# timoblak/sq-recovery

Hardware: NVIDIA B200
Metric: fused SQ implicit-loss fwd+bwd throughput (higher is better)
Workload: dtype f32

## Files before the change

sq_recovery_b200/counting.py:

```python
from __future__ import annotations

import ctypes
import os

import torch

from . import _lib
from .functional import nearest_offsets

LIB_COUNT = os.path.join(_lib.HERE, "libsqloss_count.so")
_h = None

XU_PER_EVENT = {"plane_steps": 11, "spot_backward_blocks": 5, "dealout_rounds": 13, "refine_rounds": 11,
                "column_groups": 16, "items": 6}
NAMES = ("plane_steps", "spot_backward_blocks", "dealout_rounds", "refine_rounds", "items", "column_groups",
         "queued_points", "refined_points")


def lib():
    global _h
    if _h is None:
        if not os.path.exists(LIB_COUNT):
            raise RuntimeError(f"{LIB_COUNT} not found: python -m sq_recovery_b200.build")
        h = ctypes.CDLL(LIB_COUNT)
        for name, (res, args) in _lib._PROTOS.items():
            fn = getattr(h, name)
            fn.restype, fn.argtypes = res, args
        h.sq_debug_counters.restype = ctypes.c_int
        h.sq_debug_counters.argtypes = [ctypes.c_void_p, ctypes.c_int]
        _h = h
    return _h


def implicit_counts(images: torch.Tensor, pred: torch.Tensor, n: int, tau: float, sharpness: float, want_grad: bool = True):
    h = lib()
    dev = pred.device
    B = pred.shape[0]
    p = pred.detach().float().contiguous()
    img = images.detach().float().contiguous()
    row_off, col_off = nearest_offsets(img.shape[2], img.shape[3], n, dev)
    nb = h.sq_scratch_bytes(B, n)
    scratch = torch.zeros(nb, dtype=torch.uint8, device=dev)
    loss = torch.empty((), dtype=torch.float64, device=dev)
    grad = torch.empty_like(p) if want_grad else None
    P = lambda t: ctypes.c_void_p(t.data_ptr()) if t is not None else None
    cnt = (ctypes.c_ulonglong * 8)()
    torch.cuda.synchronize()
    _lib.check(h.sq_debug_counters(cnt, 1), "sq_debug_counters")
    rc = h.sq_implicit_loss(P(p), _lib.SQ_F32, B, n, 1.0 / (n - 1), 1e-4, P(img), img.shape[2] * img.shape[3], P(row_off),
                            P(col_off), tau, sharpness, P(loss), None, P(grad), None, P(scratch), nb,
                            torch.cuda.current_stream(dev).cuda_stream)
    _lib.check(rc, "sq_implicit_loss (counting build)")
    torch.cuda.synchronize()
    _lib.check(h.sq_debug_counters(cnt, 1), "sq_debug_counters")
    c = dict(zip(NAMES, (int(v) for v in cnt)))
    grid_points = B * n ** 3
    xu = sum(XU_PER_EVENT[k] * c[k] for k in XU_PER_EVENT)
    return {"counters": c, "grid_points": grid_points, "point_evaluations": 32 * c["plane_steps"],
            "walked_fraction": 32 * c["plane_steps"] / grid_points, "xu_warp_inst_model": xu,
            "loss": loss.item()}
```

sq_recovery_b200/csrc/sq_core.cuh:

```cuda
#pragma once
#include <math.h>
#include <stdint.h>
#include <string.h>

#if defined(__CUDACC__)
#define SQ_HD __host__ __device__ __forceinline__
#else
#define SQ_HD inline
#endif

#if !defined(__CUDACC__)
struct float2 { float x, y; };
#endif

#ifndef SQ_COUNT_HOOK
#define SQ_COUNT_HOOK(i, n) do { } while (0)
#endif

namespace sq {

constexpr float kLog2e = 1.4426950408889634f;
constexpr double kLn2 = 0.6931471805599453;
constexpr float kAbsFix = 1e-2f;
#ifndef SQ_KACTIVE
// ... 37 lines not shown
#else
    return log2f(fabsf(x));
#endif
}
SQ_HD float ex2_neg_abs(float x) {
#if defined(__CUDA_ARCH__)
    float y; asm("{\n .reg .f32 t;\n abs.f32 t, %1;\n neg.f32 t, t;\n ex2.approx.ftz.f32 %0, t;\n}" : "=f"(y) : "f"(x)); return y;
#else
    return exp2f(-fabsf(x));
#endif
}

struct Grid {
    int n;
    double step;
    double z0;
    float inv_n;
    float stepf, z0f;
};
SQ_HD Grid make_grid(int n, double step, double z0) {
    Grid g; g.n = n; g.step = step; g.z0 = z0; g.inv_n = 1.0f / (float)n; g.stepf = (float)step; g.z0f = (float)z0; return g;
}
SQ_HD double grid_coord(const Grid& g, int i) { return i == 0 ? g.z0 : (double)i * g.step; }
SQ_HD float grid_coord_f32(const Grid& g, int i) { return i == 0 ? g.z0f : (float)i * g.stepf; }

SQ_HD float d2f(double v) {
#if defined(__CUDA_ARCH__)
    float y; asm("cvt.rn.f32.f64 %0, %1;" : "=f"(y) : "d"(v)); return y;
#else
    return (float)v;
#endif
}
SQ_HD double f2d(float v) {
#if defined(__CUDA_ARCH__)
    double y; asm("cvt.f64.f32 %0, %1;" : "=d"(y) : "f"(v)); return y;
#else
    return (double)v;
#endif
}

struct Sample {
    double Ms[9];
    double t[3];
    float mf[6];
    float of[3];
    float dh[3], dl[3];
    float idh[3];
    float cf0;
    float pxy, pz;
    float e21, e1;
    float wd[3];
    float qw, qa, qia, qB1;
    int zpack;
    double pxy64, pz64, e21_64, e1_64;
};
struct SampleFull : Sample {
    double M[9];
    double a[3], e[2], q[4];
    double ia[3];
    double hp[8], hrn;
    int heads, pad2_;
    float mask[8];
};

SQ_HD void split2(double v, float& hi, float& lo) { hi = d2f(v); lo = d2f(v - f2d(hi)); }

SQ_HD void heads_forward(const double* raw, double* p, double* hp, double& hrn) {
    for (int i = 0; i < 8; ++i) { hp[i] = (double)(float)(1.0 / (1.0 + exp(-raw[i]))); p[i] = hp[i]; }
    const double n2 = raw[8] * raw[8] + raw[9] * raw[9] + raw[10] * raw[10] + raw[11] * raw[11];
    hrn = 1.0 / sqrt(n2);
    for (int i = 8; i < 12; ++i) p[i] = (double)(float)(raw[i] * hrn);
}
SQ_HD void heads_backward(const double* hp, double hrn, const double* q, double* gr) {
    for (int i = 0; i < 8; ++i) gr[i] *= hp[i] * (1.0 - hp[i]);
    const double dot = q[0] * gr[8] + q[1] * gr[9] + q[2] * gr[10] + q[3] * gr[11];
    for (int i = 0; i < 4; ++i) gr[8 + i] = (gr[8 + i] - q[i] * dot) * hrn;
}

SQ_HD double clamped_param(const double* p, bool clamp, int i, float* mask = nullptr) {
    const double lo = i < 3 ? 0.05 : (i < 5 ? 0.1 : 0.0);
    double x = p[i];
    float m = 1.0f;
    if (clamp) {
        if (x < lo) { x = lo; m = 0.0f; }
        if (x > 1.0) { x = 1.0; m = 0.0f; }
    }
    if (mask) *mask = m;
    return x;
}
SQ_HD void prep_part(const double* p, bool clamp, const Grid& g, SampleFull& S, int part) {
    if (part < 3) {
        const int i = part;
        const double x = -p[8], y = -p[9], z = -p[10], w = p[11];
        const double tx = 2.0 * x, ty = 2.0 * y, tz = 2.0 * z;
        const double twx = tx * w, twy = ty * w, twz = tz * w;
        const double txx = tx * x, txy = ty * x, txz = tz * x;
        const double tyy = ty * y, tyz = tz * y, tzz = tz * z;
        double m0, m1, m2;
        if (i == 0)      { m0 = 1.0 - (tyy + tzz); m1 = txy - twz;         m2 = txz + twy; }
        else if (i == 1) { m0 = txy + twz;         m1 = 1.0 - (txx + tzz); m2 = tyz - twx; }
        else             { m0 = txz - twy;         m1 = tyz + twx;         m2 = 1.0 - (txx + tyy); }
        S.M[3 * i] = m0; S.M[3 * i + 1] = m1; S.M[3 * i + 2] = m2;
        const double a = clamped_param(p, clamp, i);
        const double t0 = clamped_param(p, clamp, 5), t1 = clamped_param(p, clamp, 6), t2 = clamped_param(p, clamp, 7);
        const double ia = 1.0 / a;
        S.ia[i] = ia;
        const double s0 = m0 * ia, s1 = m1 * ia, s2 = m2 * ia;
        S.Ms[3 * i] = s0; S.Ms[3 * i + 1] = s1; S.Ms[3 * i + 2] = s2;
        split2(s2 * g.step, S.dh[i], S.dl[i]);
        S.idh[i] = 1.0f / S.dh[i];
        S.mf[2 * i] = (float)s0; S.mf[2 * i + 1] = (float)s1;
        S.of[i] = (float)-(s0 * t0 + s1 * t1 + s2 * t2);
    } else {
        const double e1 = clamped_param(p, clamp, 3), e2 = clamped_param(p, clamp, 4);
        const double w1 = e2 > 0.0 ? (e2 < 1.0 ? exp2(e2 - 1.0) : 1.0) : 0.0;
        const double b1 = e1 > 0.0 ? (e1 < 1.0 ? exp2(1.0 - e1) : 1.0) : 1e30;
        S.qw = (float)w1; S.qB1 = (float)b1;
        S.pxy64 = 2.0 / e2; S.pz64 = 2.0 / e1; S.e21_64 = e2 / e1; S.e1_64 = e1;
        S.pxy = (float)S.pxy64; S.pz = (float)S.pz64; S.e21 = (float)S.e21_64; S.e1 = (float)e1;
        S.cf0 = (float)(g.z0 / g.step);
    }
}
SQ_HD int zero_planes(const SampleFull& S, const Grid& g) {
    int pack = 0;
    for (int i = 0; i < 3; ++i) {
        if (S.M[3 * i] != 0.0 || S.M[3 * i + 1] != 0.0 || S.M[3 * i + 2] == 0.0) continue;
        const double m = S.M[3 * i + 2], target = m * S.t[2];
        const int c0 = (int)(S.t[2] / g.step + 0.5);
        for (int c = c0 - 1; c <= c0 + 1; ++c) {
            if (c < 1 || c >= g.n || c > 1023) continue;
            if (m * grid_coord(g, c) == target) pack |= c << (10 * i);
        }
    }
    return pack;
}
SQ_HD float round13(float v) {
    int b;
#if defined(__CUDA_ARCH__)
    b = __float_as_int(v);
#else
    memcpy(&b, &v, 4);
#endif
    b = (b + 0x400) & ~0x7ff;
#if defined(__CUDA_ARCH__)
    return __int_as_float(b);
#else
    float r; memcpy(&r, &b, 4); return r;
#endif
}
SQ_HD void resplit_zero_rows(SampleFull& S, const Grid& g) {
    for (int i = 0; i < 3; ++i) {
        if (!((S.zpack >> (10 * i)) & 1023)) continue;
        const double d = S.Ms[3 * i + 2] * g.step;
        S.dh[i] = round13(d2f(d));
        S.dl[i] = round13(d2f(d - f2d(S.dh[i])));
        S.idh[i] = 1.0f / S.dh[i];
    }
}

SQ_HD void prep_finish(const double* p, bool clamp, const Grid& g, SampleFull& S) {
    for (int i = 0; i < 8; ++i) {
        float m;
        const double v = clamped_param(p, clamp, i, &m);
        S.mask[i] = m;
        if (i < 3) S.a[i] = v; else if (i < 5) S.e[i - 3] = v; else S.t[i - 5] = v;
    }
    for (int i = 0; i < 4; ++i) S.q[i] = p[8 + i];
    S.zpack = zero_planes(S, g);
    if (S.zpack) resplit_zero_rows(S, g);
    S.heads = 0; S.pad2_ = 0; S.hrn = 1.0;
    for (int i = 0; i < 8; ++i) S.hp[i] = 0.0;
    double al = 0.0;
    for (int i = 0; i < 3; ++i) {
// ... 326 lines not shown
    {
        const float r = sqrtf(bound * bound * 1.004f * S.qB1) + sqrtf(he2);
        const float beta = fmaf(S.wd[0], bc[0], fmaf(S.wd[1], bc[1], S.wd[2] * bc[2]));
        const float gamma = fmaf(S.qw, fmaf(bc[0], bc[0], bc[1] * bc[1]), fmaf(bc[2], bc[2], -r * r));
        const float disc = fmaf(beta, beta, -S.qa * gamma);
        const float sq = sqrtf(fmaxf(disc, 0.0f));
        lo = fmaxf(lo, (-beta - sq) * S.qia);
        hi = fminf(hi, disc > 0.0f ? (sq - beta) * S.qia : -1e30f);
    }
    const float nf = (float)g.n;
    lo = fminf(fmaxf(lo - 1.0f, 0.0f), nf);
    hi = fmaxf(fminf(hi + 1.0f, nf - 1.0f), -1.0f);
    const int c_lo = (int)ceilf(lo), c_hi = (int)floorf(hi);
    if (range_lo) *range_lo = c_lo;
    return c_hi >= c_lo ? c_hi - c_lo + 1 : 0;
}

SQ_HD int footprint_walk(const Sample& S, const Grid& g, float bound, float die, float cx, float cy, float hx, float hy) {
    int c_lo = 0;
    const int planes = footprint_planes(S, g, bound, cx, cy, hx, hy, &c_lo);
    if (planes <= 0 || !(die > 0.f)) return planes;
    const float a = fmaf(S.dh[0], S.dh[0], fmaf(S.dh[1], S.dh[1], S.dh[2] * S.dh[2])), ia = 1.0f / a, nf = (float)(g.n - 1);
    float stop = 1e30f;
    for (int k = 0; k < 4; ++k) {
        const float gx = (cx + ((k & 1) ? hx : -hx)) * g.stepf, gy = (cy + ((k & 2) ? hy : -hy)) * g.stepf;
        float b[3];
        for (int i = 0; i < 3; ++i) b[i] = fmaf(S.mf[2 * i], gx, fmaf(S.mf[2 * i + 1], gy, S.of[i]));
        const float beta = fmaf(S.dh[0], b[0], fmaf(S.dh[1], b[1], S.dh[2] * b[2]));
        const float gamma = fmaf(b[0], b[0], fmaf(b[1], b[1], fmaf(b[2], b[2], -0.97f)));
        const float disc = fmaf(beta, beta, -a * gamma);
        float s = (float)c_lo;
        if (disc > 0.f) {
            const float sq = sqrtf(disc);
            const float far_ = fmaxf((-beta - sq) * ia, 0.f), near_ = fminf((sq - beta) * ia, nf);
            if (near_ - far_ >= die) s = fmaxf(near_ - die - 1.0f, (float)c_lo);
        }
        stop = fminf(stop, s);
    }
    const int cut = (int)(stop - (float)c_lo);
    return cut > 0 ? (planes - cut > 1 ? planes - cut : 1) : planes;
}

SQ_HD void xfast_group_footprint(int n, int group, float& cx, float& cy, float& hx, float& hy) {
    const int first = group * 32;
    int last = first + 31;
    if (last > n * n - 1) last = n * n - 1;
    const int ib0 = first / n, ia0 = first - ib0 * n, ib1 = last / n, ia1 = last - ib1 * n;
    if (ib1 == ib0) { cx = 0.5f * (float)(ia0 + ia1); hx = 0.5f * (float)(ia1 - ia0); cy = (float)ib0; hy = 0.f; }
    else { cx = 0.5f * (float)(n - 1); hx = cx; cy = 0.5f * (float)(ib0 + ib1); hy = 0.5f * (float)(ib1 - ib0); }
}

#if defined(__CUDA_ARCH__)
#define SQ_ANY(p) __any_sync(0xffffffffu, (p))
#define SQ_BALLOT(p) __ballot_sync(0xffffffffu, (p))
#define SQ_WARP_MAX(v) __reduce_max_sync(0xffffffffu, (v))
#define SQ_WARP_MIN(v) __reduce_min_sync(0xffffffffu, (v))
#else
#define SQ_ANY(p) (p)
#define SQ_BALLOT(p) ((p) ? 1u : 0u)
#define SQ_WARP_MAX(v) (v)
#define SQ_WARP_MIN(v) (v)
#endif
SQ_HD unsigned lanes_below() {
#if defined(__CUDA_ARCH__)
    unsigned m; asm("mov.u32 %0, %%lanemask_lt;" : "=r"(m)); return m;
#else
    return 0u;
#endif
}
SQ_HD int popcount(unsigned m) {
#if defined(__CUDA_ARCH__)
    return __popc(m);
#else
    return __builtin_popcount(m);
#endif
}

SQ_HD void warp_range(int n, int& c_lo, int& c_hi) {
    const bool empty = c_hi < c_lo;
    c_hi = SQ_WARP_MAX(empty ? -1 : c_hi);
    c_lo = SQ_WARP_MIN(empty ? n : c_lo);
    if (c_hi < c_lo) { c_lo = 0; c_hi = -1; }
}

SQ_HD bool column_zero_possible(const Sample& S, const float* bh) {
    bool m = false;
    for (int i = 0; i < 3; ++i) {
        const float cs = -bh[i] * S.idh[i];
        const float r = cs - rintf(cs);
        m = m || !(fabsf(r) > 1e-4f) || !(fabsf(cs - S.cf0) > 1e-4f);
    }
    return m;
}

struct ImplicitParams { float kl; float tl; float bound; float kact; };
SQ_HD float implicit_active_bits(float kl, int n, int batch) {
    const float band = (260.0f * kLog2e / kl) * ((float)n / 64.0f);
    float bits = kActive + (band > 1.0f ? log2f(band) : 0.0f);
    const float point = log2f(kl * 1e9f / ((float)n * (float)n * (float)(batch > 0 ? batch : 1)));
    if (point > bits) bits = point;
    return bits < kImplicitCullBits ? bits : kImplicitCullBits;
}

#ifndef SQ_KDEEP
#define SQ_KDEEP 32.0f
#endif
constexpr float kDeep = SQ_KDEEP;

struct ColGrad {
    float gs0[3], gs1[3], gz0[3], gz1[3], ge0[2], ge1[2];
};

struct BwdQueue {
    float* cf;
    float* pre;
    float* x;
    float* d;
    int cap;
    int lane;
    unsigned where;
};
constexpr int kNoLink = 255;
constexpr unsigned kTagMask = 0x1fffu;
constexpr int kPoolMaxPlanes = 1024;

SQ_HD unsigned f32_bits(float v) {
#if defined(__CUDA_ARCH__)
    return __float_as_uint(v);
#else
    unsigned u; memcpy(&u, &v, 4); return u;
#endif
}
SQ_HD float bits_f32(unsigned u) {
#if defined(__CUDA_ARCH__)
    return __uint_as_float(u);
#else
    float v; memcpy(&v, &u, 4); return v;
#endif
}
SQ_HD float entry_cf(const Sample& S, float tagged) {
    const float cf = bits_f32(f32_bits(tagged) & ~kTagMask);
    return cf < 1.0f ? S.cf0 : cf;
}
SQ_HD int entry_lane(float tagged) { return (int)(f32_bits(tagged) & 31u); }
SQ_HD int entry_link(float tagged) { return (int)((f32_bits(tagged) >> 5) & 255u); }

struct ColState {
    float csl, cssum, tsum, psh, seen, T;
    BwdQueue q;
    int nr, top, head;
    bool spilled;
};

#if !defined(SQ_NO_BWD_COMPACT) && !defined(SQ_BWD_COMPACT)
// ... 106 lines not shown
                    if (active) {
#if defined(__CUDA_ARCH__)
                        const unsigned lane_ = st.q.where & 31u;
                        const int rank = popcount((shell ? ms : mp) & ((1u << lane_) - 1u));
                        const int at = shell ? st.nr + rank : st.top - rank;
                        const unsigned tag = lane_ | ((unsigned)(shell ? st.head : kNoLink) << 5);
                        const unsigned addr = (st.q.where & ~31u) + 4u * (unsigned)at;
                        asm volatile("st.shared.b32 [%0], %1;\n\tst.shared.f32 [%0 + %4], %2;\n\tst.shared.f32 [%0 + %5], %3;"
                                     :: "r"(addr), "r"((f32_bits(p.cf) & ~kTagMask) | tag), "f"(st.psh),
                                        "f"(shell ? p.x : p.eo * p.o * p.o), "n"(4 * kBwdPool), "n"(8 * kBwdPool) : "memory");
#else
                        const int rank = popcount((shell ? ms : mp) & lanes_below());
                        const int at = shell ? st.nr + rank : st.top - rank;
                        const unsigned tag = (unsigned)st.q.lane | ((unsigned)(shell ? st.head : kNoLink) << 5);
                        st.q.cf[at] = bits_f32((f32_bits(p.cf) & ~kTagMask) | tag);
                        st.q.pre[at] = st.psh;
                        st.q.x[at] = shell ? p.x : p.eo * p.o * p.o;
#endif
                        st.head = shell ? at : st.head;
                        st.seen = 1.0f;
                    }
                    st.nr = nr1; st.top = top1;
                    now = false; any_now = false;
                } else {
                    st.spilled = st.spilled || active;
                }
            }
            if (any_now)
#endif
            {
#if defined(__CUDA_ARCH__)
                SQ_COUNT_HOOK(1, 1);
#endif
                const float W = now ? p.eo * p.o * p.o : 0.0f;
                Fwd fa = p.f;
                if (!now) fwd_neutral(fa);
                Bwd b;
                point_backward<FIX>(fa, W, b);
                st.seen = now ? 1.0f : st.seen;
                const float pp = st.psh;
                for (int i = 0; i < 3; ++i) {
                    cg.gs0[i] += b.gs[i];            cg.gs1[i] = fmaf(pp, b.gs[i], cg.gs1[i]);
                    const float gz = b.gs[i] * p.cf;
                    cg.gz0[i] += gz;                 cg.gz1[i] = fmaf(pp, gz, cg.gz1[i]);
                }
                for (int i = 0; i < 2; ++i) { cg.ge0[i] += b.ge[i]; cg.ge1[i] = fmaf(pp, b.ge[i], cg.ge1[i]); }
            }
        }
        st.psh = fmaf(st.seen, st.T, st.psh);
    }
    st.tsum += st.T;
}

SQ_HD void queue_store_refined(const BwdQueue& q, int at, float x0, float x1) {
    const float eo = ex2(x1), o = rcp(1.0f + eo), w = eo * o * o;
    q.x[at] = w;
    q.d[at] = -(float)kLn2 * w * (x1 - x0);
}
SQ_HD void queue_refine_entry(const Sample& S, double step, float kl, const BwdQueue& q, int at,
                              double b0, double b1, double b2, const RefTabs& tb) {
    const float x0 = q.x[at];
    queue_store_refined(q, at, x0, refined_x(S, step, kl, b0, b1, b2, entry_cf(S, q.cf[at]), tb));
}
SQ_HD float queue_suffix_weight(const BwdQueue& q, int at, int head, float U, float tau) {
    const float Se = U - q.pre[at];
    const unsigned cfe = f32_bits(q.cf[at]) | kTagMask;
    float a = 0.f, b = 0.f;
    for (int r = head; r != kNoLink; ) {
        const float tagged = q.cf[r], d = q.d[r], Sr = U - q.pre[r];
        if ((f32_bits(tagged) | kTagMask) >= cfe) a += d; else b = fmaf(d, Sr, b);
        r = entry_link(tagged);
    }
    return Se - tau * fmaf(a, Se, b);
}
SQ_HD float queue_depth_shift(const BwdQueue& q, int head, float U) {
    float acc = 0.f;
    for (int r = head; r != kNoLink; r = entry_link(q.cf[r])) acc = fmaf(q.d[r], U - q.pre[r], acc);
    return acc;
}
template <bool FIX>
SQ_HD void queue_entry_backward(const Sample& S, const float* bh, const float* bl, float cf,
                                float w, float Sw, float sign, bool has, Bwd& b) {
    Fwd f;
    float sx = fmaf(cf, S.dh[0], bh[0]) + fmaf(cf, S.dl[0], bl[0]), sy = fmaf(cf, S.dh[1], bh[1]) + fmaf(cf, S.dl[1], bl[1]),
          sz = fmaf(cf, S.dh[2], bh[2]) + fmaf(cf, S.dl[2], bl[2]);
    point_forward<FIX>(S, sx, sy, sz, f);
    float W = w * Sw * sign;
    if (!has) { fwd_neutral(f); W = 0.f; }
    point_backward<FIX>(f, W, b);
}

#ifndef SQ_IMP_ILP
#define SQ_IMP_ILP 2
#endif

template <bool BWD, bool FIX = true, bool QUEUE = false>
SQ_HD float implicit_column(const Sample& S, const Grid& g, const ImplicitParams& P,
                            const float* bh, const float* bl, int c_lo, int c_hi, int lane_lo, float* colgrad11,
                            const BwdQueue* bwd_q = nullptr, float* U_out = nullptr, int* nr_io = nullptr, int* top_io = nullptr,
                            bool* spilled_out = nullptr, int* head_out = nullptr) {
    ColState st;
    if (QUEUE) { st.q = *bwd_q; st.nr = *nr_io; st.top = *top_io; }
    else { st.q.cf = st.q.pre = st.q.x = st.q.d = nullptr; st.q.cap = 0; st.q.lane = 0; st.q.where = 0u; st.nr = 0; st.top = -1; }
    st.spilled = false; st.head = kNoLink;
    st.csl = 0.f;
    st.T = 1.0f;
    st.tsum = (float)(g.n - 1 - c_hi);
    st.cssum = 0.f;
    st.psh = 0.f; st.seen = 0.f;
    ColGrad cg;
    if (BWD) {
        for (int i = 0; i < 3; ++i) cg.gs0[i] = cg.gs1[i] = cg.gz0[i] = cg.gz1[i] = 0.f;
        cg.ge0[0] = cg.ge0[1] = cg.ge1[0] = cg.ge1[1] = 0.f;
    }
    int c = c_hi;
    float cfi = (float)c_hi;
    bool stop = false;
#if SQ_IMP_ILP >= 2
    for (; !stop && c - (SQ_IMP_ILP - 1) >= c_lo; c -= SQ_IMP_ILP, cfi -= (float)SQ_IMP_ILP) {
        Plane p[SQ_IMP_ILP];
#if defined(__CUDA_ARCH__) && SQ_F32X2 && SQ_IMP_ILP == 2
        if (SQ_F32X2 >= 2 || !BWD) {
            plane_forward2<FIX>(S, P, bh, bl, cfi, (c - 1 == 0) ? S.cf0 : cfi - 1.0f, p[0], p[1]);
        } else
#endif
        {
#if defined(__CUDA_ARCH__)
#pragma unroll
#endif
            for (int j = 0; j < SQ_IMP_ILP; ++j)
                plane_forward<FIX>(S, P, bh, bl, (j > 0 && c - j == 0) ? S.cf0 : cfi - (float)j, p[j]);
        }
#if defined(__CUDA_ARCH__)
#pragma unroll
#endif
        for (int j = 0; j < SQ_IMP_ILP; ++j) plane_scan<BWD, FIX, QUEUE>(P, p[j], st, cg);
#ifndef SQ_NO_EARLY_EXIT
        stop = !SQ_ANY(st.csl > -kDeep && c - SQ_IMP_ILP >= lane_lo);
#endif
    }
#endif
    for (; !stop && c >= c_lo; --c, cfi -= 1.0f) {
        Plane p0;
        plane_forward<FIX>(S, P, bh, bl, (c == 0) ? S.cf0 : cfi, p0);
        plane_scan<BWD, FIX, QUEUE>(P, p0, st, cg);
#ifndef SQ_NO_EARLY_EXIT
        stop = !SQ_ANY(st.csl > -kDeep && c - 1 >= lane_lo);
#endif
    }
    const float nb = (float)(c + 1);
    st.tsum = fmaf(nb, st.T, st.tsum);
    st.cssum = fmaf(nb, st.csl, st.cssum);
    if (BWD) {
        const float U = fmaf(nb * st.seen, st.T, st.psh);
        if (QUEUE) { *U_out = U; *nr_io = st.nr; *top_io = st.top; *spilled_out = st.spilled; *head_out = st.head; }
        for (int i = 0; i < 3; ++i) {
            colgrad11[i]     = fmaf(U, cg.gs0[i], -cg.gs1[i]);
            colgrad11[3 + i] = fmaf(U, cg.gz0[i], -cg.gz1[i]);
            colgrad11[6 + i] = fmaf(bh[i], colgrad11[i], fmaf(S.dh[i], colgrad11[3 + i],
                               fmaf(bl[i], colgrad11[i], S.dl[i] * colgrad11[3 + i])));
        }
        colgrad11[9]  = fmaf(U, cg.ge0[0], -cg.ge1[0]);
        colgrad11[10] = fmaf(U, cg.ge0[1], -cg.ge1[1]);
    }
    const float depth = fmaf(-st.tsum, g.inv_n, 1.0f);
    return depth < 1e-4f ? -(float)kLn2 * st.cssum * g.inv_n : depth;
}

SQ_HD void implicit_fold(Acc& acc, const float* colgrad11, float w, float dx, float dy) {
    for (int i = 0; i < 3; ++i) {
        const float gsi = w * colgrad11[i];
        acc.gs[i] += gsi;
        acc.gm[3 * i + 0] = fmaf(gsi, dx, acc.gm[3 * i + 0]);
        acc.gm[3 * i + 1] = fmaf(gsi, dy, acc.gm[3 * i + 1]);
        acc.gm[3 * i + 2] = fmaf(w, colgrad11[3 + i], acc.gm[3 * i + 2]);
        acc.wa[i] = fmaf(w, colgrad11[6 + i], acc.wa[i]);
    }
    acc.ge[0] = fmaf(w, colgrad11[9], acc.ge[0]);
    acc.ge[1] = fmaf(w, colgrad11[10], acc.ge[1]);
}

SQ_HD void acc_add_point(Acc& acc, const Bwd& b, float cf, float dx, float dy) {
    for (int i = 0; i < 3; ++i) {
        acc.gs[i] += b.gs[i];
        acc.gm[3 * i + 0] = fmaf(b.gs[i], dx, acc.gm[3 * i + 0]);
        acc.gm[3 * i + 1] = fmaf(b.gs[i], dy, acc.gm[3 * i + 1]);
        acc.gm[3 * i + 2] = fmaf(b.gs[i], cf, acc.gm[3 * i + 2]);
        acc.wa[i] += b.wa[i];
    }
    acc.ge[0] += b.ge[0]; acc.ge[1] += b.ge[1];
}

// ... 242 lines not shown
```

sq_recovery_b200/csrc/sqloss.cu:

```cuda
#include <cuda_runtime.h>
#include <stdint.h>
#include <stdio.h>
#include <string.h>
#include <new>

#include "../../include/sqloss.h"
#ifdef SQ_TIMELINE
__device__ unsigned long long g_bwd_stats[2];
#endif
#if defined(SQ_TIMELINE) && defined(SQ_BWD_STATS)
#define SQ_BWD_HOOK(a) do { const unsigned m_ = __ballot_sync(0xffffffffu, (a)); if ((threadIdx.x & 31) == 0) { \
    atomicAdd(&g_bwd_stats[0], 1ull); atomicAdd(&g_bwd_stats[1], (unsigned long long)__popc(m_)); } } while (0)
#endif
#ifdef SQ_ITEMLOG
__device__ float g_planlog[4 * 65536];
__device__ int g_itemlog[4 * 65536];
#endif
#ifdef SQ_COUNT
__device__ unsigned long long g_count[8];
#define SQ_COUNT_HOOK(i, n) do { if ((threadIdx.x & 31) == 0) atomicAdd(&g_count[i], (unsigned long long)(n)); } while (0)
#else
#define SQ_COUNT_HOOK(i, n) do { } while (0)
#endif
#include "sq_core.cuh"

using namespace sq;

namespace {

#ifndef SQ_IMPB_THREADS
#define SQ_IMPB_THREADS 128
#endif
#ifndef SQ_IMPB_MINB
#define SQ_IMPB_MINB 5
#endif
#ifndef SQ_TILE_ALIAS
#define SQ_TILE_ALIAS 1
#endif
#ifndef SQ_WALK_ESTIMATE
#define SQ_WALK_ESTIMATE 1
#endif
#ifndef SQ_DENSE_ILP
#define SQ_DENSE_ILP 1
#endif
#ifndef SQ_IMPB_CPT
#define SQ_IMPB_CPT 1
#endif
#ifndef SQ_IMPF_THREADS
#define SQ_IMPF_THREADS 256
#endif
#ifndef SQ_IMPF_MINB
#define SQ_IMPF_MINB 4
#endif
#ifndef SQ_IMPF_CPT
#define SQ_IMPF_CPT 1
#endif
#ifndef SQ_EXP_THREADS
#define SQ_EXP_THREADS 256
#endif
#ifndef SQ_EXP_MINB
#define SQ_EXP_MINB 2
#endif
#ifndef SQ_EXP_CPT
#define SQ_EXP_CPT 1
#endif
#ifndef SQ_IOU_THREADS
#define SQ_IOU_THREADS 128
#endif
#ifndef SQ_IOU_MINB
#define SQ_IOU_MINB 4
#endif
#ifndef SQ_IOU_CPT
// ... 1345 lines not shown
    if (dev >= 0 && dev < 64 && !opted[dev]) {
        const cudaError_t e = cudaFuncSetAttribute(KERNEL, cudaFuncAttributeMaxDynamicSharedMemorySize, (int)dyn);
        if (e != cudaSuccess) return e;
        opted[dev] = true;
    }
    return cudaSuccess;
}

int launch_prep(const void* params, int dtype, int batch, bool clamp, const Grid& g, SampleFull* out, Control* ctl,
                cudaStream_t st) {
    if (dtype != SQ_F32 && dtype != SQ_F64) return (int)cudaErrorInvalidValue;
    prep_kernel<<<(batch + 3) / 4, 128, 0, st>>>(params, dtype, batch, clamp ? 1 : 0, g, out, ctl);
    return (int)cudaGetLastError();
}

struct PlanTarget { const float* target; long long tstride; const int* row_off; const int* col_off; };

int launch_plan(const void* params_a, const void* params_b, int dtype, int batch, bool clamp, const Grid& g,
                const Layout& L, float bound, const Scratch& s, unsigned long long* counts, unsigned char* item_class,
                const PlanTarget* pt, cudaStream_t st, bool heads = false, float die = 0.f) {
    if (dtype != SQ_F32 && dtype != SQ_F64) return (int)cudaErrorInvalidValue;
    int* queue = L.rows_per_sample <= kPlanMaxItems ? s.queue : nullptr;
    const PlanTarget none{nullptr, 0, nullptr, nullptr};
    const PlanTarget& t = pt ? *pt : none;
    const bool small = batch > 4 * device_sm_count();
    if (params_b) {
        auto k = small ? plan_kernel<2, kPlanThreadsSmall> : plan_kernel<2, kPlanThreads>;
        k<<<batch, small ? kPlanThreadsSmall : kPlanThreads, 0, st>>>(params_a, params_b, dtype, clamp ? 1 : 0, 0, g, L, bound, 0.f, s.tru, s.pred,
                                                                      s.ctl, counts, queue, s.queue_cap, queue ? item_class : nullptr,
                                                                      nullptr, 0, nullptr, nullptr, nullptr);
    } else {
        auto k = small ? plan_kernel<1, kPlanThreadsSmall> : plan_kernel<1, kPlanThreads>;
        k<<<batch, small ? kPlanThreadsSmall : kPlanThreads, 0, st>>>(params_a, nullptr, dtype, clamp ? 1 : 0, heads ? 1 : 0, g, L, bound, die, s.pred,
                                                                      nullptr, s.ctl, counts, queue, s.queue_cap, queue ? item_class : nullptr,
                                                                      t.target, t.tstride, t.row_off, t.col_off, pt ? s.tv_sum : nullptr);
    }
    return (int)cudaGetLastError();
}

}

extern "C" {

const char* sq_version(void) { return "sqloss-b200 0.1 (sm_100a)"; }

const char* sq_error_string(int err) { return cudaGetErrorString((cudaError_t)err); }

int sq_device_sm_count(int device, int* sm_count) {
    return (int)cudaDeviceGetAttribute(sm_count, cudaDevAttrMultiProcessorCount, device);
}

#ifdef SQ_COUNT
int sq_debug_counters(unsigned long long* host_out, int reset) {
    cudaError_t e = cudaMemcpyFromSymbol(host_out, g_count, sizeof(unsigned long long) * 8);
    if (e == cudaSuccess && reset) {
        const unsigned long long zero[8] = {0, 0, 0, 0, 0, 0, 0, 0};
        e = cudaMemcpyToSymbol(g_count, zero, sizeof zero);
    }
    return (int)e;
}
#endif

#ifdef SQ_ITEMLOG
int sq_debug_itemlog(float* plan_out, int* item_out, int n) {
    int rc = (int)cudaMemcpyFromSymbol(plan_out, g_planlog, sizeof(float) * 4 * (size_t)n);
    if (!rc) rc = (int)cudaMemcpyFromSymbol(item_out, g_itemlog, sizeof(int) * 4 * (size_t)n);
    return rc;
}
#endif
#ifdef SQ_PHASES
int sq_debug_phases(unsigned long long* host_out, int reset) {
    int rc = (int)cudaMemcpyFromSymbol(host_out, g_phase, sizeof(unsigned long long) * 8);
    if (!rc && reset) { unsigned long long z[8] = {0, 0, 0, 0, 0, 0, 0, 0}; rc = (int)cudaMemcpyToSymbol(g_phase, z, sizeof z); }
    return rc;
}
#endif
#ifdef SQ_TIMELINE
int sq_debug_timeline(unsigned long long* host_out, int n) {
    return (int)cudaMemcpyFromSymbol(host_out, g_timeline, sizeof(unsigned long long) * 3 * (size_t)n);
}
int sq_debug_bwd(unsigned long long* host_out) {
    return (int)cudaMemcpyFromSymbol(host_out, g_bwd_stats, sizeof(unsigned long long) * 2);
}
int sq_debug_plan(unsigned long long* host_out) {
    return (int)cudaMemcpyFromSymbol(host_out, g_plan_ts, sizeof(unsigned long long) * 16);
}
int sq_debug_classes(unsigned int* host_out) {
    return (int)cudaMemcpyFromSymbol(host_out, g_classes, sizeof(unsigned int) * kClasses);
}
#endif

void sq_profile_events(void* ev_before, void* ev_after) {
    t_ev_before = static_cast<cudaEvent_t>(ev_before);
    t_ev_after = static_cast<cudaEvent_t>(ev_after);
}

size_t sq_scratch_bytes(int batch, int n) {
    if (batch <= 0 || n <= 0) return 0;
    return scratch_layout(batch, n, nullptr, nullptr);
}

int sq_scratch_init(void* scratch, size_t scratch_bytes, sq_stream_t stream) {
    if (!scratch || scratch_bytes < sizeof(Control)) return (int)cudaErrorInvalidValue;
    return (int)cudaMemsetAsync(scratch, 0, sizeof(Control), static_cast<cudaStream_t>(stream));
}

static int implicit_loss_impl(const void* pred, int pred_dtype, int batch, int n, double step, double z0,
                              const float* target, long long target_stride_b, const int* row_off, const int* col_off,
                              float tau, float sharpness, double* loss_out, double* per_sample, void* grad_pred,
                              float* depth_out, void* scratch, size_t scratch_bytes, sq_stream_t stream, bool heads) {
    Scratch s;
    int rc = check_scratch(batch, n, scratch, scratch_bytes, &s);
    if (rc) return rc;
    if (target && (!row_off || !col_off)) return (int)cudaErrorInvalidValue;
    if (grad_pred && !target) return (int)cudaErrorInvalidValue;
    cudaStream_t st = static_cast<cudaStream_t>(stream);
    const Grid g = make_grid(n, step, z0);
    const Layout L = make_layout(n, grad_pred ? SQ_IMPB_CPT : SQ_IMPF_CPT);
    const ImplicitParams P{sharpness * kLog2e, tau * kLog2e, implicit_cull_bound(sharpness * kLog2e), implicit_active_bits(sharpness * kLog2e, n, batch)};
    if (depth_out)
        SQ_TRY(cudaMemsetAsync(depth_out, 0, sizeof(float) * (size_t)batch * n * n, st));
#ifdef SQ_SKIP_COLUMN
    SQ_TRY(cudaMemsetAsync(s.ctl, 0, sizeof(Control), st));
#endif
    const PlanTarget pt{target, target_stride_b, row_off, col_off};
    rc = launch_plan(pred, nullptr, pred_dtype, batch, true, g, L, P.bound, s, nullptr, target ? s.item_class : nullptr,
                     target ? &pt : nullptr, st, heads, SQ_WALK_ESTIMATE ? 32.0f / P.tl : 0.f);
    if (rc) return rc;
    const int items = batch * L.rows_per_sample;
    const int* queue = L.rows_per_sample <= kPlanMaxItems ? s.queue : nullptr;
#ifdef SQ_PDL
    const bool pdl = (t_ev_before == nullptr && t_ev_after == nullptr);
#else
    const bool pdl = false;
#endif
#ifndef SQ_SKIP_COLUMN
    {
        ColumnKernelTimer timer(st);
        if (grad_pred) {
            const int blocks = persistent_blocks(items, SQ_IMPB_THREADS / 32, SQ_IMPB_MINB);
            constexpr size_t dyn = kImplicitBwdSmemPerWarp * (SQ_IMPB_THREADS / 32);
            SQ_TRY((opt_in_dyn_smem<implicit_kernel<true, SQ_IMPB_THREADS, SQ_IMPB_MINB, SQ_IMPB_CPT>>(dyn)));
            SQ_TRY(launch_dependent(implicit_kernel<true, SQ_IMPB_THREADS, SQ_IMPB_MINB, SQ_IMPB_CPT>, blocks, SQ_IMPB_THREADS, dyn, st, pdl,
                                    s.pred, g, L, P, items, s.ctl, queue, s.queue_cap, target, target_stride_b, row_off, col_off,
                                    s.partials, depth_out));
        } else {
            const int blocks = persistent_blocks(items, SQ_IMPF_THREADS / 32, SQ_IMPF_MINB);
            SQ_TRY(launch_dependent(implicit_kernel<false, SQ_IMPF_THREADS, SQ_IMPF_MINB, SQ_IMPF_CPT>, blocks, SQ_IMPF_THREADS, 0, st, pdl,
                                    s.pred, g, L, P, items, s.ctl, queue, s.queue_cap, target, target_stride_b, row_off, col_off,
                                    s.partials, depth_out));
        }
    }
    SQ_TRY(cudaGetLastError());
#endif
#ifndef SQ_SKIP_FINALIZE
    if (target) {
        const double nn = (double)n * n;
        SQ_TRY(launch_dependent(finalize_kernel<FIN_IMPLICIT>, batch, kFinThreads, 0, st, pdl,
                                s.pred, g, batch, L.rows_per_sample, s.partials, 1.0 / nn,
                                -(double)sharpness * (double)tau / (nn * n * (double)batch), pred_dtype, grad_pred, s.per_sample,
                                per_sample, loss_out, &s.ctl->ticket, s.tv_sum, queue ? s.item_class : nullptr));
        SQ_TRY(cudaGetLastError());
    }
#endif
    return 0;
}

int sq_implicit_loss(const void* pred, int pred_dtype, int batch, int n, double step, double z0,
                     const float* target, long long target_stride_b, const int* row_off, const int* col_off,
                     float tau, float sharpness, double* loss_out, double* per_sample, void* grad_pred,
                     float* depth_out, void* scratch, size_t scratch_bytes, sq_stream_t stream) {
    return implicit_loss_impl(pred, pred_dtype, batch, n, step, z0, target, target_stride_b, row_off, col_off, tau, sharpness,
                              loss_out, per_sample, grad_pred, depth_out, scratch, scratch_bytes, stream, false);
}

int sq_implicit_loss_heads(const void* raw_heads, int dtype, int batch, int n, double step, double z0,
                           const float* target, long long target_stride_b, const int* row_off, const int* col_off,
                           float tau, float sharpness, double* loss_out, double* per_sample, void* grad_raw,
                           float* depth_out, void* scratch, size_t scratch_bytes, sq_stream_t stream) {
    return implicit_loss_impl(raw_heads, dtype, batch, n, step, z0, target, target_stride_b, row_off, col_off, tau, sharpness,
                              loss_out, per_sample, grad_raw, depth_out, scratch, scratch_bytes, stream, true);
}

int sq_depth_projection_vjp(const void* pred, int pred_dtype, int batch, int n, double step, double z0,
                            float tau, float sharpness, const float* grad_depth, void* grad_pred,
                            void* scratch, size_t scratch_bytes, sq_stream_t stream) {
    Scratch s;
    int rc = check_scratch(batch, n, scratch, scratch_bytes, &s);
    if (rc) return rc;
    if (!grad_depth || !grad_pred) return (int)cudaErrorInvalidValue;
    cudaStream_t st = static_cast<cudaStream_t>(stream);
    const Grid g = make_grid(n, step, z0);
    const Layout L = make_layout(n, SQ_IMPB_CPT);
    const ImplicitParams P{sharpness * kLog2e, tau * kLog2e, implicit_cull_bound(sharpness * kLog2e), implicit_active_bits(sharpness * kLog2e, n, 1)};
    rc = launch_plan(pred, nullptr, pred_dtype, batch, true, g, L, P.bound, s, nullptr, s.item_class, nullptr, st, false,
                     SQ_WALK_ESTIMATE ? 32.0f / P.tl : 0.f);
    if (rc) return rc;
    const int items = batch * L.rows_per_sample;
    const int* queue = L.rows_per_sample <= kPlanMaxItems ? s.queue : nullptr;
#ifdef SQ_PDL
    const bool pdl = (t_ev_before == nullptr && t_ev_after == nullptr);
#else
    const bool pdl = false;
#endif
    {
        ColumnKernelTimer timer(st);
        const int blocks = persistent_blocks(items, SQ_IMPB_THREADS / 32, SQ_IMPB_MINB);
        constexpr size_t dyn = kImplicitBwdSmemPerWarp * (SQ_IMPB_THREADS / 32);
        SQ_TRY((opt_in_dyn_smem<implicit_kernel<true, SQ_IMPB_THREADS, SQ_IMPB_MINB, SQ_IMPB_CPT, true>>(dyn)));
        SQ_TRY(launch_dependent(implicit_kernel<true, SQ_IMPB_THREADS, SQ_IMPB_MINB, SQ_IMPB_CPT, true>, blocks, SQ_IMPB_THREADS, dyn,
                                st, pdl, s.pred, g, L, P, items, s.ctl, queue, s.queue_cap, grad_depth, 0LL,
                                static_cast<const int*>(nullptr), static_cast<const int*>(nullptr), s.partials,
                                static_cast<float*>(nullptr)));
    }
    SQ_TRY(cudaGetLastError());
    SQ_TRY(launch_dependent(finalize_kernel<FIN_IMPLICIT>, batch, kFinThreads, 0, st, pdl,
                            s.pred, g, batch, L.rows_per_sample, s.partials, 0.0, -(double)sharpness * (double)tau / (double)n,
                            pred_dtype, grad_pred, s.per_sample, static_cast<double*>(nullptr), static_cast<double*>(nullptr),
                            &s.ctl->ticket, static_cast<const double*>(nullptr), queue ? s.item_class : nullptr));
    SQ_TRY(cudaGetLastError());
    return 0;
}

int sq_explicit_loss(const void* true_params, const void* pred, int params_dtype, int batch, int n, double step,
                     double z0, float sharpness, float mult, double* loss_out, double* per_sample, void* grad_pred,
                     void* scratch, size_t scratch_bytes, sq_stream_t stream) {
    Scratch s;
    int rc = check_scratch(batch, n, scratch, scratch_bytes, &s);
    if (rc) return rc;
    if (!true_params || !pred) return (int)cudaErrorInvalidValue;
    cudaStream_t st = static_cast<cudaStream_t>(stream);
    const Grid g = make_grid(n, step, z0);
    const Layout L = make_layout(n, SQ_EXP_CPT);
    const float kl = sharpness * kLog2e, bound = cull_bound_bits(kl, 24.0f);
    rc = launch_plan(true_params, pred, params_dtype, batch, true, g, L, bound, s, nullptr, s.item_class, nullptr, st);
    if (rc) return rc;
    const int items = batch * L.rows_per_sample;
    const int* queue = L.rows_per_sample <= kPlanMaxItems ? s.queue : nullptr;
    const int blocks = persistent_blocks(items, SQ_EXP_THREADS / 32, SQ_EXP_MINB);
    {
        ColumnKernelTimer timer(st);
        if (grad_pred) explicit_kernel<true><<<blocks, SQ_EXP_THREADS, 0, st>>>(s.tru, s.pred, g, L, kl, bound, items, s.ctl, queue, s.queue_cap, s.partials);
        else explicit_kernel<false><<<blocks, SQ_EXP_THREADS, 0, st>>>(s.tru, s.pred, g, L, kl, bound, items, s.ctl, queue, s.queue_cap, s.partials);
    }
    SQ_TRY(cudaGetLastError());
    const double n3 = (double)n * n * n;
    finalize_kernel<FIN_EXPLICIT><<<batch, kFinThreads, 0, st>>>(
// ... 387 lines not shown
```

Before: 1359.

## Skip per-plane SDF evaluation through convex superquadric interiors with probed run-ahead

When every lane in a warp sits deep inside a convex superquadric (e1, e2 <= 1), the column walk probes a plane further down. If that plane is also deep interior for all lanes, it advances over the whole run with a cheap constant-slope transmittance update and skips evaluating the implicit function per plane. Probe distances are halved on failure, and the interior threshold is set from the active-bits bound. This relies on convexity, so that two deep-interior planes imply the planes between them are deep interior too. It adds probe evaluations and warp votes, and an environment variable can turn the path off.

```diff
diff --git a/sq_recovery_b200/counting.py b/sq_recovery_b200/counting.py
--- a/sq_recovery_b200/counting.py
+++ b/sq_recovery_b200/counting.py
@@ -12,9 +12,9 @@
 _h = None
 
 XU_PER_EVENT = {"plane_steps": 11, "spot_backward_blocks": 5, "dealout_rounds": 13, "refine_rounds": 11,
-                "column_groups": 16, "items": 6}
+                "column_groups": 16, "items": 6, "interior_steps": 1 - 11, "interior_probes": 10}
 NAMES = ("plane_steps", "spot_backward_blocks", "dealout_rounds", "refine_rounds", "items", "column_groups",
-         "queued_points", "refined_points")
+         "queued_points", "refined_points", "interior_steps", "interior_probes")
 
 
 def lib():
@@ -44,7 +44,7 @@
     loss = torch.empty((), dtype=torch.float64, device=dev)
     grad = torch.empty_like(p) if want_grad else None
     P = lambda t: ctypes.c_void_p(t.data_ptr()) if t is not None else None
-    cnt = (ctypes.c_ulonglong * 8)()
+    cnt = (ctypes.c_ulonglong * len(NAMES))()
     torch.cuda.synchronize()
     _lib.check(h.sq_debug_counters(cnt, 1), "sq_debug_counters")
     rc = h.sq_implicit_loss(P(p), _lib.SQ_F32, B, n, 1.0 / (n - 1), 1e-4, P(img), img.shape[2] * img.shape[3], P(row_off),
@@ -57,5 +57,6 @@
     grid_points = B * n ** 3
     xu = sum(XU_PER_EVENT[k] * c[k] for k in XU_PER_EVENT)
     return {"counters": c, "grid_points": grid_points, "point_evaluations": 32 * c["plane_steps"],
-            "walked_fraction": 32 * c["plane_steps"] / grid_points, "xu_warp_inst_model": xu,
+            "walked_fraction": 32 * c["plane_steps"] / grid_points,
+            "interior_fraction": c["interior_steps"] / c["plane_steps"] if c["plane_steps"] else 0.0, "xu_warp_inst_model": xu,
             "loss": loss.item()}
diff --git a/sq_recovery_b200/csrc/sq_core.cuh b/sq_recovery_b200/csrc/sq_core.cuh
--- a/sq_recovery_b200/csrc/sq_core.cuh
+++ b/sq_recovery_b200/csrc/sq_core.cuh
@@ -113,6 +113,7 @@
     float wd[3];
     float qw, qa, qia, qB1;
     int zpack;
+    int convex;
     double pxy64, pz64, e21_64, e1_64;
 };
 struct SampleFull : Sample {
@@ -180,6 +181,7 @@
         S.pxy64 = 2.0 / e2; S.pz64 = 2.0 / e1; S.e21_64 = e2 / e1; S.e1_64 = e1;
         S.pxy = (float)S.pxy64; S.pz = (float)S.pz64; S.e21 = (float)S.e21_64; S.e1 = (float)e1;
         S.cf0 = (float)(g.z0 / g.step);
+        S.convex = (e1 > 0.0 && e1 <= 1.0 && e2 > 0.0 && e2 <= 1.0) ? 1 : 0;
     }
 }
 SQ_HD int zero_planes(const SampleFull& S, const Grid& g) {
@@ -612,11 +614,13 @@
 
 #if defined(__CUDA_ARCH__)
 #define SQ_ANY(p) __any_sync(0xffffffffu, (p))
+#define SQ_ALL(p) __all_sync(0xffffffffu, (p))
 #define SQ_BALLOT(p) __ballot_sync(0xffffffffu, (p))
 #define SQ_WARP_MAX(v) __reduce_max_sync(0xffffffffu, (v))
 #define SQ_WARP_MIN(v) __reduce_min_sync(0xffffffffu, (v))
 #else
 #define SQ_ANY(p) (p)
+#define SQ_ALL(p) (p)
 #define SQ_BALLOT(p) ((p) ? 1u : 0u)
 #define SQ_WARP_MAX(v) (v)
 #define SQ_WARP_MIN(v) (v)
@@ -653,13 +657,26 @@
     return m;
 }
 
-struct ImplicitParams { float kl; float tl; float bound; float kact; };
+#ifndef SQ_INTERIOR_XOFF
+#define SQ_INTERIOR_XOFF 0.0f
+#endif
+struct ImplicitParams {
+    float kl, tl, bound, kact;
+    float xoff = SQ_INTERIOR_XOFF;
+};
 SQ_HD float implicit_active_bits(float kl, int n, int batch) {
     const float band = (260.0f * kLog2e / kl) * ((float)n / 64.0f);
     float bits = kActive + (band > 1.0f ? log2f(band) : 0.0f);
     const float point = log2f(kl * 1e9f / ((float)n * (float)n * (float)(batch > 0 ? batch : 1)));
     if (point > bits) bits = point;
     return bits < kImplicitCullBits ? bits : kImplicitCullBits;
+}
+
+SQ_HD float interior_threshold(float kact) { return fmaxf(kact, 24.5f) + 1.0f; }
+
+SQ_HD ImplicitParams implicit_params(float sharpness, float tau, int n, int batch) {
+    const float kl = sharpness * kLog2e, kact = implicit_active_bits(kl, n, batch);
+    return ImplicitParams{kl, tau * kLog2e, implicit_cull_bound(kl), kact};
 }
 
 #ifndef SQ_KDEEP
@@ -872,6 +889,21 @@
     st.tsum += st.T;
 }
 
+template <bool BWD>
+SQ_HD void plane_scan_interior(const ImplicitParams& P, ColState& st) {
+#if defined(__CUDA_ARCH__)
+    SQ_COUNT_HOOK(0, 1);
+#endif
+#if defined(__CUDA_ARCH__) || !defined(__CUDACC__)
+    SQ_COUNT_HOOK(8, 1);
+#endif
+    st.csl = fmaf(1.0f, -P.tl, st.csl);
+    st.cssum += st.csl;
+    st.T = ex2(st.csl);
+    if (BWD) st.psh = fmaf(st.seen, st.T, st.psh);
+    st.tsum += st.T;
+}
+
 SQ_HD void queue_store_refined(const BwdQueue& q, int at, float x0, float x1) {
     const float eo = ex2(x1), o = rcp(1.0f + eo), w = eo * o * o;
     q.x[at] = w;
@@ -913,6 +945,7 @@
 #ifndef SQ_IMP_ILP
 #define SQ_IMP_ILP 2
 #endif
+constexpr int kRunMin = 4;
 
 template <bool BWD, bool FIX = true, bool QUEUE = false>
 SQ_HD float implicit_column(const Sample& S, const Grid& g, const ImplicitParams& P,
@@ -936,6 +969,8 @@
     int c = c_hi;
     float cfi = (float)c_hi;
     bool stop = false;
+    const float xin = interior_threshold(P.kact) + P.xoff;
+    int fail = c_lo - 1;
 #if SQ_IMP_ILP >= 2
     for (; !stop && c - (SQ_IMP_ILP - 1) >= c_lo; c -= SQ_IMP_ILP, cfi -= (float)SQ_IMP_ILP) {
         Plane p[SQ_IMP_ILP];
@@ -958,6 +993,31 @@
 #ifndef SQ_NO_EARLY_EXIT
         stop = !SQ_ANY(st.csl > -kDeep && c - SQ_IMP_ILP >= lane_lo);
 #endif
+        if (!stop && SQ_ALL(p[SQ_IMP_ILP - 1].x <= -xin) && S.convex) {
+            const float planes = fminf(fmaxf((st.csl + kDeep) * rcp(P.tl), 0.0f), (float)g.n);
+            int m = SQ_WARP_MAX((int)ceilf(planes * (1.0f / SQ_IMP_ILP)));
+            const int room = (c - SQ_IMP_ILP - fail) / SQ_IMP_ILP;
+            m = m < room ? m : room;
+            for (; m * SQ_IMP_ILP >= kRunMin; m >>= 1) {
+                const int cp = c - SQ_IMP_ILP * (m + 1) + 1;
+                Plane pr;
+                plane_forward<FIX>(S, P, bh, bl, (cp == 0) ? S.cf0 : (float)cp, pr);
+#if defined(__CUDA_ARCH__) || !defined(__CUDACC__)
+                SQ_COUNT_HOOK(9, 1);
+#endif
+                if (SQ_ALL(pr.x <= -xin)) {
+                    do {
+                        c -= SQ_IMP_ILP; cfi -= (float)SQ_IMP_ILP;
+                        for (int j = 0; j < SQ_IMP_ILP; ++j) plane_scan_interior<BWD>(P, st);
+#ifndef SQ_NO_EARLY_EXIT
+                        stop = !SQ_ANY(st.csl > -kDeep && c - SQ_IMP_ILP >= lane_lo);
+#endif
+                    } while (!stop && c - SQ_IMP_ILP + 1 > cp);
+                    break;
+                }
+                fail = cp;
+            }
+        }
     }
 #endif
     for (; !stop && c >= c_lo; --c, cfi -= 1.0f) {
diff --git a/sq_recovery_b200/csrc/sqloss.cu b/sq_recovery_b200/csrc/sqloss.cu
--- a/sq_recovery_b200/csrc/sqloss.cu
+++ b/sq_recovery_b200/csrc/sqloss.cu
@@ -1,6 +1,7 @@
 #include <cuda_runtime.h>
 #include <stdint.h>
 #include <stdio.h>
+#include <stdlib.h>
 #include <string.h>
 #include <new>
 
@@ -17,7 +18,7 @@
 __device__ int g_itemlog[4 * 65536];
 #endif
 #ifdef SQ_COUNT
-__device__ unsigned long long g_count[8];
+__device__ unsigned long long g_count[10];
 #define SQ_COUNT_HOOK(i, n) do { if ((threadIdx.x & 31) == 0) atomicAdd(&g_count[i], (unsigned long long)(n)); } while (0)
 #else
 #define SQ_COUNT_HOOK(i, n) do { } while (0)
@@ -1469,9 +1470,9 @@
 
 #ifdef SQ_COUNT
 int sq_debug_counters(unsigned long long* host_out, int reset) {
-    cudaError_t e = cudaMemcpyFromSymbol(host_out, g_count, sizeof(unsigned long long) * 8);
+    cudaError_t e = cudaMemcpyFromSymbol(host_out, g_count, sizeof g_count);
     if (e == cudaSuccess && reset) {
-        const unsigned long long zero[8] = {0, 0, 0, 0, 0, 0, 0, 0};
+        const unsigned long long zero[10] = {};
         e = cudaMemcpyToSymbol(g_count, zero, sizeof zero);
     }
     return (int)e;
@@ -1520,6 +1521,13 @@
 int sq_scratch_init(void* scratch, size_t scratch_bytes, sq_stream_t stream) {
     if (!scratch || scratch_bytes < sizeof(Control)) return (int)cudaErrorInvalidValue;
     return (int)cudaMemsetAsync(scratch, 0, sizeof(Control), static_cast<cudaStream_t>(stream));
+}
+
+static ImplicitParams implicit_params_env(float sharpness, float tau, int n, int batch) {
+    ImplicitParams P = implicit_params(sharpness, tau, n, batch);
+    const char* e = getenv("SQ_INTERIOR_RUN");
+    if (e && e[0] == '0') P.xoff = INFINITY;
+    return P;
 }
 
 static int implicit_loss_impl(const void* pred, int pred_dtype, int batch, int n, double step, double z0,
@@ -1534,7 +1542,7 @@
     cudaStream_t st = static_cast<cudaStream_t>(stream);
     const Grid g = make_grid(n, step, z0);
     const Layout L = make_layout(n, grad_pred ? SQ_IMPB_CPT : SQ_IMPF_CPT);
-    const ImplicitParams P{sharpness * kLog2e, tau * kLog2e, implicit_cull_bound(sharpness * kLog2e), implicit_active_bits(sharpness * kLog2e, n, batch)};
+    const ImplicitParams P = implicit_params_env(sharpness, tau, n, batch);
     if (depth_out)
         SQ_TRY(cudaMemsetAsync(depth_out, 0, sizeof(float) * (size_t)batch * n * n, st));
 #ifdef SQ_SKIP_COLUMN
@@ -1609,7 +1617,7 @@
     cudaStream_t st = static_cast<cudaStream_t>(stream);
     const Grid g = make_grid(n, step, z0);
     const Layout L = make_layout(n, SQ_IMPB_CPT);
-    const ImplicitParams P{sharpness * kLog2e, tau * kLog2e, implicit_cull_bound(sharpness * kLog2e), implicit_active_bits(sharpness * kLog2e, n, 1)};
+    const ImplicitParams P = implicit_params_env(sharpness, tau, n, 1);
     rc = launch_plan(pred, nullptr, pred_dtype, batch, true, g, L, P.bound, s, nullptr, s.item_class, nullptr, st, false,
                      SQ_WALK_ESTIMATE ? 32.0f / P.tl : 0.f);
     if (rc) return rc;
```

Result: slower. 1317, median of 6 (-3.1%).
